# VITA-Group/CV_A-FAN

Measured on AMD Instinct MI355X. Metric: images/sec (whole node) A-FAN K=5 train step, ResNet-18/CIFAR-10, higher is better.
Workload: dtype bf16; 1 GPU; resnet18 CIFAR-10-shape A-FAN K=5 bf16, batch 256/GPU, perturb_idx 6, internal layout nhwc, 1xMI355X per rank (BASELINE configs[1]); global_batch=256, parallelism=dp1, hipgraph=True, in_launch_batchnorm=True

## Files before the change

### cv_a-fan_amd/csrc/afan_wgrad.hip

```cpp
#include "afan_common.h"
#include "afan_conv_stem.h"
#include "afan_wgrad_small.h"
#include <stdlib.h>

using namespace afan;

namespace {

typedef __bf16 bf16x8 __attribute__((ext_vector_type(8)));
typedef short s16x4 __attribute__((ext_vector_type(4)));
typedef float f32x16 __attribute__((ext_vector_type(16)));
typedef uint32_t u32x4 __attribute__((ext_vector_type(4)));

constexpr int THREADS = 256;
constexpr int BKP = 64;

struct FastDiv {
    uint32_t m, l;
};
static FastDiv make_fastdiv(uint32_t d) {
    FastDiv f;
    uint32_t l = 0;
    while ((1u << l) < d) ++l;
    f.l = l;
    f.m = (uint32_t)((((uint64_t)1 << 32) * (((uint64_t)1 << l) - d)) / d + 1);
    return f;
}
__device__ __forceinline__ uint32_t fdiv(uint32_t x, FastDiv f) { return (__umulhi(x, f.m) + x) >> f.l; }

struct WgradP {
    const uint16_t* x;
    const uint16_t* dy;
    float* slab;
    int N, Hi, Wi, Ci, Ho, Wo, Co;
    int k, stride, pad, dil;
    int S;
    int steps_per_slice;
    uint32_t P;
    FastDiv dWo, dHo;
    const uint16_t* x2;
    const uint16_t* dy2;
    uint32_t P1;
    int N2;
    int dn, dho, N1;
    int xcd_remap;
    float* direct;
    int accumulate;
};

template <int BM, int BN, bool INC>
__device__ __forceinline__ void wgrad_body(const WgradP& p, const uint32_t lin, const uint32_t tiles_, const uint32_t taps_,
                                           const uint32_t total) {
    constexpr int TM = BM / 2, TN = BN / 2, MI = TM / 32, NI = TN / 32;
    constexpr int LDA = BM + 32, LDB = BN + 32;
    constexpr int PA = BM / 8, PB = BN / 8;
    constexpr int RA = THREADS / PA, RB = THREADS / PB;
    constexpr int NA = BKP / RA, NB = BKP / RB;
    __shared__ __attribute__((aligned(16))) uint16_t As[BKP * LDA];
    __shared__ __attribute__((aligned(16))) uint16_t Bs[BKP * LDB];

    const int tid = threadIdx.x, lane = tid & 63, wave = tid >> 6;
    const int wr = wave >> 1, wc = wave & 1;
    const int tiles_n = (p.Ci + BN - 1) / BN;
    int tap, slice, tile;
    {
        uint32_t logical = lin;
        if (p.xcd_remap) {
            const uint32_t per = total >> 3, main_ = per << 3;
            if (lin < main_) logical = (lin & 7u) * per + (lin >> 3);
        }
        tap = (int)(logical % taps_);
        const uint32_t rest = logical / taps_;
        tile = (int)(rest % tiles_);
        slice = (int)(rest / tiles_);
    }
    const int co0 = (tile / tiles_n) * BM, ci0 = (tile % tiles_n) * BN;
    const int dh = (tap / p.k) * p.dil - p.pad, dw = (tap % p.k) * p.dil - p.pad;

    const __amdgpu_buffer_rsrc_t xr = __builtin_amdgcn_make_buffer_rsrc(
        const_cast<uint16_t*>(p.x), 0, (int)((int64_t)p.N * p.Hi * p.Wi * p.Ci * 2), 0x00020000);
    const __amdgpu_buffer_rsrc_t dr = __builtin_amdgcn_make_buffer_rsrc(
        const_cast<uint16_t*>(p.dy), 0, (int)((int64_t)p.P1 * p.Co * 2), 0x00020000);
    const __amdgpu_buffer_rsrc_t xr2 = __builtin_amdgcn_make_buffer_rsrc(
        const_cast<uint16_t*>(p.x2), 0, p.x2 ? (int)((int64_t)p.N2 * p.Hi * p.Wi * p.Ci * 2) : 0, 0x00020000);
    const __amdgpu_buffer_rsrc_t dr2 = __builtin_amdgcn_make_buffer_rsrc(
        const_cast<uint16_t*>(p.dy2), 0, p.dy2 ? (int)((int64_t)(p.P - p.P1) * p.Co * 2) : 0, 0x00020000);
    constexpr uint32_t OOB = 0x80000000u;

    const int pa = tid % PA, ra0 = tid / PA;
    const int pb = tid % PB, rb0 = tid / PB;
    const bool a_ok = co0 + pa * 8 < p.Co, b_ok = ci0 + pb * 8 < p.Ci;
    const uint32_t p_begin = (uint32_t)slice * p.steps_per_slice * BKP;

    f32x16 acc[MI][NI];
#pragma unroll
    for (int i = 0; i < MI; ++i)
#pragma unroll
        for (int j = 0; j < NI; ++j)
#pragma unroll
            for (int r = 0; r < 16; ++r) acc[i][j][r] = 0.f;

    u32x4 va[NA], vb[NB];
    int rn[NB], rho[NB];
    bool wi_ok[NB];
    uint32_t col_off[NB];
    if constexpr (INC) {
#pragma unroll
        for (int i = 0; i < NB; ++i) {
            const uint32_t pix = p_begin + rb0 + i * RB;
            const uint32_t t1 = fdiv(pix, p.dWo), wo = pix - t1 * p.Wo;
            const uint32_t n = fdiv(t1, p.dHo);
            rn[i] = (int)n;
            rho[i] = (int)(t1 - n * p.Ho);
            const int wi = (int)wo * p.stride + dw;
            wi_ok[i] = wi >= 0 && wi < p.Wi;
            col_off[i] = (uint32_t)((wi * p.Ci + ci0 + pb * 8) * 2);
        }
    }
    auto gload = [&](int ks) {
        const uint32_t pbase = p_begin + ks * BKP;
        const bool seg2 = pbase >= p.P1;
        const uint32_t shift = seg2 ? p.P1 : 0u, plim = seg2 ? p.P : p.P1;
        const __amdgpu_buffer_rsrc_t dsel = seg2 ? dr2 : dr, xsel = seg2 ? xr2 : xr;
#pragma unroll
        for (int i = 0; i < NA; ++i) {
            const uint32_t pix = pbase + ra0 + i * RA;
            const uint32_t off = (pix < plim && a_ok) ? ((pix - shift) * p.Co + co0 + pa * 8) * 2u : OOB;
            va[i] = __builtin_bit_cast(u32x4, __builtin_amdgcn_raw_buffer_load_b128(dsel, (int)off, 0, 0));
        }
#pragma unroll
        for (int i = 0; i < NB; ++i) {
            const uint32_t pix = pbase + rb0 + i * RB;
            if constexpr (INC) {
                const int hi = rho[i] * p.stride + dh;
                const int nl = rn[i] - (seg2 ? p.N1 : 0);
                const bool ok = pix < plim && wi_ok[i] && hi >= 0 && hi < p.Hi && b_ok;
                const uint32_t off = ok ? ((uint32_t)((nl * p.Hi + hi) * p.Wi) * (uint32_t)p.Ci) * 2u + col_off[i] : OOB;
                vb[i] = __builtin_bit_cast(u32x4, __builtin_amdgcn_raw_buffer_load_b128(xsel, (int)off, 0, 0));
                rn[i] += p.dn;
                rho[i] += p.dho;
                if (rho[i] >= p.Ho) { rho[i] -= p.Ho; rn[i] += 1; }
            } else {
                const uint32_t pl = pix - shift;
                const uint32_t t1 = fdiv(pl, p.dWo), wo = pl - t1 * p.Wo;
                const uint32_t n = fdiv(t1, p.dHo), ho = t1 - n * p.Ho;
                const int hi = (int)ho * p.stride + dh, wi = (int)wo * p.stride + dw;
                const bool ok = pix < plim && hi >= 0 && hi < p.Hi && wi >= 0 && wi < p.Wi && b_ok;
                const uint32_t off = ok ? (((n * p.Hi + hi) * p.Wi + wi) * p.Ci + ci0 + pb * 8) * 2u : OOB;
                vb[i] = __builtin_bit_cast(u32x4, __builtin_amdgcn_raw_buffer_load_b128(xsel, (int)off, 0, 0));
            }
        }
    };
    auto lstore = [&]() {
#pragma unroll
        for (int i = 0; i < NA; ++i) *reinterpret_cast<u32x4*>(As + (ra0 + i * RA) * LDA + pa * 8) = va[i];
#pragma unroll
        for (int i = 0; i < NB; ++i) *reinterpret_cast<u32x4*>(Bs + (rb0 + i * RB) * LDB + pb * 8) = vb[i];
    };
    const int fr = 8 * (lane >> 5) + ((lane & 15) >> 2);
    const int fc = 16 * ((lane >> 4) & 1) + 4 * (lane & 3);
    auto frag = [&](const uint16_t* T, int ld, int kbase, int cbase) -> bf16x8 {
        typedef s16x4 __attribute__((address_space(3))) * lptr;
        const uint16_t* a0 = T + (kbase + fr) * ld + cbase + fc;
        const s16x4 lo = __builtin_amdgcn_ds_read_tr16_b64_v4i16((lptr)(a0));
        const s16x4 hi = __builtin_amdgcn_ds_read_tr16_b64_v4i16((lptr)(a0 + 4 * ld));
        typedef short s16x8 __attribute__((ext_vector_type(8)));
        s16x8 v = {lo[0], lo[1], lo[2], lo[3], hi[0], hi[1], hi[2], hi[3]};
        return __builtin_bit_cast(bf16x8, v);
    };

    int KS = p.steps_per_slice;
    {
        const int64_t remaining = (int64_t)p.P - (int64_t)p_begin;
        const int64_t need = remaining <= 0 ? 0 : (remaining + BKP - 1) / BKP;
        if (need < KS) KS = (int)need;
    }
    if (KS > 0) gload(0);
    for (int ks = 0; ks < KS; ++ks) {
        lstore();
        __syncthreads();
        if (ks + 1 < KS) gload(ks + 1);
#pragma unroll
        for (int kk = 0; kk < BKP / 16; ++kk) {
            bf16x8 fa[MI], fb[NI];
#pragma unroll
            for (int i = 0; i < MI; ++i) fa[i] = frag(As, LDA, kk * 16, wr * TM + i * 32);
#pragma unroll
            for (int j = 0; j < NI; ++j) fb[j] = frag(Bs, LDB, kk * 16, wc * TN + j * 32);
#pragma unroll
            for (int i = 0; i < MI; ++i)
#pragma unroll
                for (int j = 0; j < NI; ++j)
                    acc[i][j] = __builtin_amdgcn_mfma_f32_32x32x16_bf16(fa[i], fb[j], acc[i][j], 0, 0, 0);
        }
        __syncthreads();
    }
    const int taps = p.k * p.k;
    float* out = p.slab + (((int64_t)slice * taps + tap) * p.Co) * p.Ci;
#pragma unroll
    for (int i = 0; i < MI; ++i)
#pragma unroll
        for (int j = 0; j < NI; ++j)
#pragma unroll
            for (int r = 0; r < 16; ++r) {
                const int co = co0 + wr * TM + i * 32 + (r & 3) + 8 * (r >> 2) + 4 * (lane >> 5);
                const int ci = ci0 + wc * TN + j * 32 + (lane & 31);
                if (co < p.Co && ci < p.Ci) {
                    if (p.direct) {
                        float* g = p.direct + ((int64_t)co * taps + tap) * p.Ci + ci;
                        *g = p.accumulate ? *g + acc[i][j][r] : acc[i][j][r];
                    } else {
                        out[(int64_t)co * p.Ci + ci] = acc[i][j][r];
                    }
                }
            }
}

template <int BM, int BN, bool INC>
__global__ __launch_bounds__(THREADS) void wgrad_kernel(const WgradP p) {
    wgrad_body<BM, BN, INC>(p, blockIdx.x + gridDim.x * (blockIdx.y + gridDim.y * blockIdx.z), gridDim.x, gridDim.y,
                            gridDim.x * gridDim.y * gridDim.z);
}

__device__ __forceinline__ f32x4 sum_slices(const float* __restrict__ p, int64_t stride, int S) {
    f32x4 s = {0.f, 0.f, 0.f, 0.f};
    int k = 0;
    for (; k + 8 <= S; k += 8) {
        f32x4 v[8];
#pragma unroll
        for (int u = 0; u < 8; ++u) v[u] = *reinterpret_cast<const f32x4*>(p + (int64_t)(k + u) * stride);
#pragma unroll
        for (int u = 0; u < 8; ++u) s += v[u];
    }
    for (; k < S; ++k) s += *reinterpret_cast<const f32x4*>(p + (int64_t)k * stride);
    return s;
}

constexpr int MAXQ = 4;
struct WgradPN {
    int n;
    uint32_t first[MAXQ + 1];
    uint32_t count[MAXQ];
    uint32_t tiles[MAXQ], taps[MAXQ];
    WgradP p[MAXQ];
};
template <int BM, int BN, bool INC>
__global__ __launch_bounds__(THREADS) void wgrad_multi_kernel(const WgradPN pn) {
    int q = 0;
    while (q + 1 < pn.n && blockIdx.x >= pn.first[q + 1]) ++q;
    const uint32_t lin = blockIdx.x - pn.first[q];
    if (lin >= pn.count[q]) return;
    wgrad_body<BM, BN, INC>(pn.p[q], lin, pn.tiles[q], pn.taps[q], pn.count[q]);
}

struct RedPN {
    const float* slab[MAXQ];
    float* grad[MAXQ];
    int S[MAXQ], taps[MAXQ], Co[MAXQ], Ci[MAXQ];
};
__global__ __launch_bounds__(THREADS) void wgrad_reduce_multi_kernel(const RedPN r, int accumulate) {
    const int q = blockIdx.y;
    const float* __restrict__ slab = r.slab[q];
    float* __restrict__ grad = r.grad[q];
    const int S = r.S[q], taps = r.taps[q], Co = r.Co[q], Ci = r.Ci[q];
    const int64_t per = (int64_t)taps * Co * Ci;
    const int64_t nvec = per / 4;
    for (int64_t v = (int64_t)blockIdx.x * THREADS + threadIdx.x; v < nvec; v += (int64_t)gridDim.x * THREADS) {
        const int64_t e = v * 4;
        const int ci = (int)(e % Ci);
        const int64_t t2 = e / Ci;
        const int co = (int)(t2 % Co);
        const int tap = (int)(t2 / Co);
        f32x4 s = sum_slices(slab + e, per, S);
        float* g = grad + ((int64_t)co * taps + tap) * Ci + ci;
        if (accumulate) s += *reinterpret_cast<const f32x4*>(g);
        *reinterpret_cast<f32x4*>(g) = s;
    }
}

__global__ __launch_bounds__(THREADS) void wgrad_reduce_kernel(const float* __restrict__ slab, float* __restrict__ grad,
                                                               int S, int taps, int Co, int Ci, int accumulate) {
    const int64_t per = (int64_t)taps * Co * Ci;
    const int64_t nvec = per / 4;
    for (int64_t v = (int64_t)blockIdx.x * THREADS + threadIdx.x; v < nvec; v += (int64_t)gridDim.x * THREADS) {
        const int64_t e = v * 4;
        const int ci = (int)(e % Ci);
        const int64_t t2 = e / Ci;
        const int co = (int)(t2 % Co);
        const int tap = (int)(t2 / Co);
        f32x4 s = sum_slices(slab + e, per, S);
        float* g = grad + ((int64_t)co * taps + tap) * Ci + ci;
        if (accumulate) s += *reinterpret_cast<const f32x4*>(g);
        *reinterpret_cast<f32x4*>(g) = s;
    }
}

struct Plan {
    int bm, bn, S, steps;
};

Plan make_plan(int64_t P, int co, int ci, int taps) {
    Plan pl;
    pl.bm = (co % 128 == 0) ? 128 : 64;
    pl.bn = (ci % 128 == 0) ? 128 : 64;
    const int64_t tiles = (int64_t)((co + pl.bm - 1) / pl.bm) * ((ci + pl.bn - 1) / pl.bn) * taps;
    const int64_t total_steps = (P + BKP - 1) / BKP;
    static const int target = [] { const char* v = getenv("AFAN_WGRAD_WGS"); return v ? atoi(v) : 512; }();
    int64_t S = target / tiles;
    static const int min_steps_env = [] { const char* v = getenv("AFAN_WGRAD_MINSTEPS"); return v ? atoi(v) : 0; }();
    const int min_steps = min_steps_env > 0 ? min_steps_env : (total_steps <= 40 ? 5 : 16);
    const int64_t max_s = total_steps / min_steps > 0 ? total_steps / min_steps : 1;
    if (S > max_s) S = max_s;
    if (S < 1) S = 1;
    static const int direct_on = [] { const char* v = getenv("AFAN_WGRAD_DIRECT"); return v ? atoi(v) : 0; }();
    if (direct_on && S == 2 && total_steps <= 64) S = 1;
    pl.steps = (int)((total_steps + S - 1) / S);
    pl.S = (int)((total_steps + pl.steps - 1) / pl.steps);
    return pl;
}

int build_problem(const void* x, const void* dy, int64_t n, const void* x2, const void* dy2, int64_t n2, float* grad, int64_t hi,
                  int64_t wi, int64_t ci, int64_t co, int k, int stride, int dilation, float* workspace, int accumulate,
                  WgradP& p, Plan& pl);

template <int BM, int BN>
int launch(const WgradP& p, int taps, hipStream_t st) {
    dim3 grid((unsigned)(((p.Co + BM - 1) / BM) * ((p.Ci + BN - 1) / BN)), (unsigned)taps, (unsigned)p.S);
    if (p.dn >= 0) wgrad_kernel<BM, BN, true><<<grid, THREADS, 0, st>>>(p);
    else wgrad_kernel<BM, BN, false><<<grid, THREADS, 0, st>>>(p);
    AFAN_LAUNCH_CHECK();
    AFAN_TRACE_LAUNCH("wgrad<%d,%d,inc%d>", BM, BN, p.dn >= 0 ? 1 : 0);
    return AFAN_OK;
}

}

extern "C" {

int64_t afan_conv_wgrad_workspace_floats(int64_t n, int64_t hi, int64_t wi, int64_t ci, int64_t co, int k, int stride) {
    if (ci == 3) return afan_stem::eligible(n, hi, wi, ci, co, k, stride) ? afan_stem::wgrad_workspace_floats(n, hi, wi, co) : 0;
    if (afan_wgrad_small::eligible(n, hi, wi, ci, co, k, stride)) return afan_wgrad_small::workspace_floats(n, hi, wi, ci, co, stride);
    if (n <= 0 || hi <= 0 || wi <= 0 || ci % 8 || co % 8 || ci < 40 || co < 40 || !(k == 1 || k == 3) || !(stride == 1 || stride == 2))
        return 0;
    const int pad = k / 2;
    const int64_t P = n * ((hi + 2 * pad - k) / stride + 1) * ((wi + 2 * pad - k) / stride + 1);
    const Plan pl = make_plan(P, (int)co, (int)ci, k * k);
    return (int64_t)pl.S * k * k * co * ci;
}

int afan_conv_wgrad_nhwc_bf16(const void* x, const void* dy, float* grad, int64_t n, int64_t hi, int64_t wi, int64_t ci,
                              int64_t co, int k, int stride, int dilation, float* workspace, int accumulate,
                              afan_stream_t stream) {
    return afan_conv_wgrad2_nhwc_bf16(x, dy, n, nullptr, nullptr, 0, grad, hi, wi, ci, co, k, stride, dilation, workspace,
                                      accumulate, stream);
}

int afan_conv_wgrad2_nhwc_bf16(const void* x, const void* dy, int64_t n, const void* x2, const void* dy2, int64_t n2,
                               float* grad, int64_t hi, int64_t wi, int64_t ci, int64_t co, int k, int stride, int dilation,
                               float* workspace, int accumulate, afan_stream_t stream) {
    if (n <= 0 || hi <= 0 || wi <= 0 || ci <= 0 || co <= 0 || n2 < 0) return AFAN_ESHAPE;
    AFAN_TRACE_PROBLEM(0, afan::trace::WGRAD, n + n2, hi, wi, ci, co, k, stride, dilation);
    if (dilation < 1 || (dilation > 1 && (k != 3 || stride != 1 || ci % 8 || co % 8 || ci < 40 || co < 40))) return AFAN_ESHAPE;
    if (n2 > 0 && ci == 3) return AFAN_ESHAPE;
    if (n2 > 0 && (!x2 || !dy2)) return AFAN_ENULL;
    if (ci == 3) {
        if (!afan_stem::eligible(n, hi, wi, ci, co, k, stride)) return AFAN_ESHAPE;
        if (!x || !dy || !grad || !workspace) return AFAN_ENULL;
        if (!aligned(dy, 16) || !aligned(grad, 4) || !aligned(workspace, 16)) return AFAN_EALIGN;
        hipStream_t st = (hipStream_t)stream;
        const double M = (double)n * hi * wi;
        AFAN_PROF_FLOPS("conv_stem_wgrad_kernel", 2.0 * (M * co + M * 3), 2.0 * M * co * 27, st);
        return afan_stem::wgrad_launch(x, dy, grad, n, hi, wi, co, workspace, accumulate, st);
    }
    if (dilation == 1 && afan_wgrad_small::eligible(n, hi, wi, ci, co, k, stride)) {
        if (!x || !dy || !grad || !workspace) return AFAN_ENULL;
        if (!aligned(x, 16) || !aligned(dy, 16) || !aligned(grad, 4) || !aligned(workspace, 16)) return AFAN_EALIGN;
        hipStream_t st = (hipStream_t)stream;
        const double P = (double)n * ((hi - 1) / stride + 1) * ((wi - 1) / stride + 1);
        AFAN_PROF_FLOPS("conv_wgrad_small_kernel", 2.0 * (P * co + (double)n * hi * wi * ci), 2.0 * P * co * ci * 9, st);
        if (n2 > 0 && (!aligned(x2, 16) || !aligned(dy2, 16))) return AFAN_EALIGN;
        return afan_wgrad_small::launch(x, dy, grad, n, hi, wi, ci, co, stride, workspace, accumulate, st, x2, dy2, n2);
    }
    WgradP p{};
    Plan pl;
    int e = build_problem(x, dy, n, x2, dy2, n2, grad, hi, wi, ci, co, k, stride, dilation, workspace, accumulate, p, pl);
    if (e) return e;
    const int taps = k * k;
    const int64_t P = (n + n2) * (int64_t)p.Ho * p.Wo;
    hipStream_t st = (hipStream_t)stream;
    int rc;
    {
        AFAN_PROF_FLOPS("conv_wgrad_kernel", 2.0 * (double)(P * co + n * hi * wi * ci) + 4.0 * pl.S * taps * co * ci,
                        2.0 * (double)P * co * ci * taps, st);
        if (pl.bm == 128) rc = pl.bn == 128 ? launch<128, 128>(p, taps, st) : launch<128, 64>(p, taps, st);
        else rc = pl.bn == 128 ? launch<64, 128>(p, taps, st) : launch<64, 64>(p, taps, st);
    }
    if (rc || p.direct) return rc;
    const int64_t per = (int64_t)taps * co * ci;
    AFAN_PROF("conv_wgrad_reduce_kernel", 4.0 * per * (pl.S + 1 + (accumulate ? 1 : 0)), st);
    wgrad_reduce_kernel<<<grid_for(per / 4, THREADS, 1024), THREADS, 0, st>>>(workspace, grad, pl.S, taps, (int)co, (int)ci,
                                                                              accumulate);
    AFAN_LAUNCH_CHECK();
    return AFAN_OK;
}

}

namespace {
int build_problem(const void* x, const void* dy, int64_t n, const void* x2, const void* dy2, int64_t n2, float* grad, int64_t hi,
                  int64_t wi, int64_t ci, int64_t co, int k, int stride, int dilation, float* workspace, int accumulate,
                  WgradP& p, Plan& pl) {
    if (ci % 8 || co % 8 || ci < 40 || co < 40 || !(k == 1 || k == 3) || !(stride == 1 || stride == 2)) return AFAN_ESHAPE;
    if (!x || !dy || !grad || !workspace) return AFAN_ENULL;
    if (!aligned(x, 16) || !aligned(dy, 16) || !aligned(grad, 16) || !aligned(workspace, 16)) return AFAN_EALIGN;
    const int pad = dilation * (k / 2);
    const int64_t ho = (hi + 2 * (k / 2) - k) / stride + 1, wo = (wi + 2 * (k / 2) - k) / stride + 1;
    const int64_t P1 = n * ho * wo, P = (n + n2) * ho * wo;
    if (P * co * 2 > 0x7fffffffLL || (n + n2) * hi * wi * ci * 2 > 0x7fffffffLL) return AFAN_ESHAPE;
    if (n2 > 0 && (P1 % BKP != 0 || !aligned(x2, 16) || !aligned(dy2, 16))) return n2 > 0 && P1 % BKP != 0 ? AFAN_ESHAPE : AFAN_EALIGN;
    const int taps = k * k;
    pl = make_plan(P, (int)co, (int)ci, taps);
    p.x = (const uint16_t*)x; p.dy = (const uint16_t*)dy; p.slab = workspace;
    p.N = (int)n; p.Hi = (int)hi; p.Wi = (int)wi; p.Ci = (int)ci; p.Ho = (int)ho; p.Wo = (int)wo; p.Co = (int)co;
    p.k = k; p.stride = stride; p.pad = pad; p.dil = dilation; p.S = pl.S; p.steps_per_slice = pl.steps; p.P = (uint32_t)P;
    p.x2 = (const uint16_t*)x2; p.dy2 = (const uint16_t*)dy2; p.P1 = (uint32_t)P1; p.N2 = (int)n2;
    p.N1 = (int)n;
    {
        static const bool remap_on = [] { const char* v = getenv("AFAN_WGRAD_XCD"); return !v || atoi(v) != 0; }();
        p.xcd_remap = remap_on ? 1 : 0;
    }
    p.dn = -1; p.dho = 0;
    {
        static const bool inc_on = [] { const char* v = getenv("AFAN_WGRAD_INC"); return !v || atoi(v) != 0; }();
        if (inc_on && BKP % wo == 0) {
            const int64_t hw = ho * wo;
            p.dn = (int)(BKP / hw);
            p.dho = (int)((BKP % hw) / wo);
        }
    }
    p.dWo = make_fastdiv((uint32_t)wo); p.dHo = make_fastdiv((uint32_t)ho);
    {
        static const int direct_on = [] { const char* v = getenv("AFAN_WGRAD_DIRECT"); return v ? atoi(v) : 0; }();
        p.direct = (direct_on && pl.S == 1) ? grad : nullptr;
        p.accumulate = accumulate;
    }
    return AFAN_OK;
}
}

extern "C" {

int afan_conv_wgrad_plan(int64_t n, int64_t hi, int64_t wi, int64_t ci, int64_t co, int k, int stride) {
    if (ci == 3 || afan_wgrad_small::eligible(n, hi, wi, ci, co, k, stride)) return 0;
    if (n <= 0 || hi <= 0 || wi <= 0 || ci % 8 || co % 8 || ci < 40 || co < 40 || !(k == 1 || k == 3) || !(stride == 1 || stride == 2))
        return 0;
    const int64_t ho = (hi + 2 * (k / 2) - k) / stride + 1, wo = (wi + 2 * (k / 2) - k) / stride + 1;
    const Plan pl = make_plan(n * ho * wo, (int)co, (int)ci, k * k);
    static const bool inc_on = [] { const char* v = getenv("AFAN_WGRAD_INC"); return !v || atoi(v) != 0; }();
    const int inc = (inc_on && BKP % wo == 0) ? 1 : 0;
    return pl.bm | (pl.bn << 8) | (inc << 16) | (1 << 17);
}

int afan_conv_wgrad_multi_nhwc_bf16(int nb, const void* const* x, const void* const* dy, float* const* grad, const int64_t* n,
                                    const int64_t* hi, const int64_t* wi, const int64_t* ci, const int64_t* co, const int* k,
                                    const int* stride, const int* dilation, float* workspace, int accumulate,
                                    afan_stream_t stream) {
    if (nb < 1 || nb > MAXQ) return AFAN_ESHAPE;
    if (!x || !dy || !grad || !n || !hi || !wi || !ci || !co || !k || !stride || !dilation || !workspace) return AFAN_ENULL;
    WgradPN pn{};
    RedPN rp{};
    pn.n = nb;
    int code0 = 0;
    int64_t woff = 0, max_vec = 0;
    double bytes = 0, flops = 0;
    for (int b = 0; b < nb; ++b) {
        const int code = afan_conv_wgrad_plan(n[b], hi[b], wi[b], ci[b], co[b], k[b], stride[b]);
        if (!code || (b && code != code0)) return AFAN_ESHAPE;
        code0 = code;
        if (dilation[b] < 1 || (dilation[b] > 1 && (k[b] != 3 || stride[b] != 1))) return AFAN_ESHAPE;
        AFAN_TRACE_PROBLEM(b, afan::trace::WGRAD, n[b], hi[b], wi[b], ci[b], co[b], k[b], stride[b], dilation[b]);
        Plan pl;
        int e = build_problem(x[b], dy[b], n[b], nullptr, nullptr, 0, grad[b], hi[b], wi[b], ci[b], co[b], k[b], stride[b],
                              dilation[b], workspace + woff, accumulate, pn.p[b], pl);
        if (e) return e;
        pn.p[b].direct = nullptr;
        const int taps = k[b] * k[b];
        const int bm = code & 0xff, bn = (code >> 8) & 0xff;
        pn.tiles[b] = (uint32_t)(((co[b] + bm - 1) / bm) * ((ci[b] + bn - 1) / bn));
        pn.taps[b] = (uint32_t)taps;
        pn.count[b] = pn.tiles[b] * taps * (uint32_t)pl.S;
        pn.first[b + 1] = (pn.first[b] + pn.count[b] + 7u) & ~7u;
        rp.slab[b] = workspace + woff; rp.grad[b] = grad[b]; rp.S[b] = pl.S; rp.taps[b] = taps; rp.Co[b] = (int)co[b]; rp.Ci[b] = (int)ci[b];
        const int64_t per = (int64_t)taps * co[b] * ci[b];
        woff += (int64_t)pl.S * per;
        if (per / 4 > max_vec) max_vec = per / 4;
        const double P = (double)n[b] * pn.p[b].Ho * pn.p[b].Wo;
        bytes += 2.0 * (P * co[b] + (double)n[b] * hi[b] * wi[b] * ci[b]) + 4.0 * pl.S * per;
        flops += 2.0 * P * co[b] * ci[b] * taps;
    }
    hipStream_t st = (hipStream_t)stream;
    const int bm = code0 & 0xff, bn = (code0 >> 8) & 0xff;
    const bool inc = (code0 >> 16) & 1;
    const unsigned G = pn.first[nb];
    {
    AFAN_PROF_FLOPS("conv_wgrad_kernel", bytes, flops, st);
#define AFAN_WM(BM_, BN_)                                                                                   \
    do {                                                                                                    \
        if (inc) wgrad_multi_kernel<BM_, BN_, true><<<G, THREADS, 0, st>>>(pn);                             \
        else wgrad_multi_kernel<BM_, BN_, false><<<G, THREADS, 0, st>>>(pn);                                \
    } while (0)
    if (bm == 128) { if (bn == 128) AFAN_WM(128, 128); else AFAN_WM(128, 64); }
    else { if (bn == 128) AFAN_WM(64, 128); else AFAN_WM(64, 64); }
#undef AFAN_WM
    AFAN_LAUNCH_CHECK();
    AFAN_TRACE_LAUNCH("wgrad_multi<%d,%d,inc%d>", bm, bn, inc ? 1 : 0);
    }
    AFAN_PROF("conv_wgrad_reduce_kernel", 4.0 * (double)woff, st);
    wgrad_reduce_multi_kernel<<<dim3((unsigned)grid_for(max_vec, THREADS, 1024), (unsigned)nb), THREADS, 0, st>>>(rp, accumulate);
    AFAN_LAUNCH_CHECK();
    return AFAN_OK;
}

}
```

Measured before the change: 33960 images/sec.

## Double-buffer LDS and register fragments in wgrad kernel; size split-K from occupancy

The wgrad MFMA kernel now keeps two LDS stages, so the next tile is stored and the one after is prefetched from global memory partway through the current tile's MFMA loop. This removes one of the two barriers per K step. LDS fragments are also double-buffered in registers, so reads for the next kk overlap the current MFMAs. The split-K workgroup target, previously a fixed 512, is now CUs times min(occupancy, 2), queried per tile shape. Doubled LDS and extra fragment registers may lower occupancy, and the getenv lookups are no longer cached statics, so they run on every plan call.

Result: slower. 33610 images/sec (-1.0%).

```diff
diff --git a/cv_a-fan_amd/csrc/afan_wgrad.hip b/cv_a-fan_amd/csrc/afan_wgrad.hip
--- a/cv_a-fan_amd/csrc/afan_wgrad.hip
+++ b/cv_a-fan_amd/csrc/afan_wgrad.hip
@@ -56,8 +56,8 @@
     constexpr int PA = BM / 8, PB = BN / 8;
     constexpr int RA = THREADS / PA, RB = THREADS / PB;
     constexpr int NA = BKP / RA, NB = BKP / RB;
-    __shared__ __attribute__((aligned(16))) uint16_t As[BKP * LDA];
-    __shared__ __attribute__((aligned(16))) uint16_t Bs[BKP * LDB];
+    __shared__ __attribute__((aligned(16))) uint16_t As[2 * BKP * LDA];
+    __shared__ __attribute__((aligned(16))) uint16_t Bs[2 * BKP * LDB];
 
     const int tid = threadIdx.x, lane = tid & 63, wave = tid >> 6;
     const int wr = wave >> 1, wc = wave & 1;
@@ -151,11 +151,13 @@
             }
         }
     };
-    auto lstore = [&]() {
-#pragma unroll
-        for (int i = 0; i < NA; ++i) *reinterpret_cast<u32x4*>(As + (ra0 + i * RA) * LDA + pa * 8) = va[i];
-#pragma unroll
-        for (int i = 0; i < NB; ++i) *reinterpret_cast<u32x4*>(Bs + (rb0 + i * RB) * LDB + pb * 8) = vb[i];
+    auto lstore = [&](int stage) {
+        uint16_t* A = As + stage * (BKP * LDA);
+        uint16_t* B = Bs + stage * (BKP * LDB);
+#pragma unroll
+        for (int i = 0; i < NA; ++i) *reinterpret_cast<u32x4*>(A + (ra0 + i * RA) * LDA + pa * 8) = va[i];
+#pragma unroll
+        for (int i = 0; i < NB; ++i) *reinterpret_cast<u32x4*>(B + (rb0 + i * RB) * LDB + pb * 8) = vb[i];
     };
     const int fr = 8 * (lane >> 5) + ((lane & 15) >> 2);
     const int fc = 16 * ((lane >> 4) & 1) + 4 * (lane & 3);
@@ -175,23 +177,38 @@
         const int64_t need = remaining <= 0 ? 0 : (remaining + BKP - 1) / BKP;
         if (need < KS) KS = (int)need;
     }
-    if (KS > 0) gload(0);
+    if (KS > 0) {
+        gload(0);
+        lstore(0);
+        if (KS > 1) gload(1);
+    }
+    __syncthreads();
     for (int ks = 0; ks < KS; ++ks) {
-        lstore();
-        __syncthreads();
-        if (ks + 1 < KS) gload(ks + 1);
+        const int cur = ks & 1;
+        const uint16_t* A = As + cur * (BKP * LDA);
+        const uint16_t* B = Bs + cur * (BKP * LDB);
+        bf16x8 fa[2][MI], fb[2][NI];
+#pragma unroll
+        for (int i = 0; i < MI; ++i) fa[0][i] = frag(A, LDA, 0, wr * TM + i * 32);
+#pragma unroll
+        for (int j = 0; j < NI; ++j) fb[0][j] = frag(B, LDB, 0, wc * TN + j * 32);
 #pragma unroll
         for (int kk = 0; kk < BKP / 16; ++kk) {
-            bf16x8 fa[MI], fb[NI];
-#pragma unroll
-            for (int i = 0; i < MI; ++i) fa[i] = frag(As, LDA, kk * 16, wr * TM + i * 32);
-#pragma unroll
-            for (int j = 0; j < NI; ++j) fb[j] = frag(Bs, LDB, kk * 16, wc * TN + j * 32);
+            if (kk + 1 < BKP / 16) {
+#pragma unroll
+                for (int i = 0; i < MI; ++i) fa[(kk + 1) & 1][i] = frag(A, LDA, (kk + 1) * 16, wr * TM + i * 32);
+#pragma unroll
+                for (int j = 0; j < NI; ++j) fb[(kk + 1) & 1][j] = frag(B, LDB, (kk + 1) * 16, wc * TN + j * 32);
+            }
 #pragma unroll
             for (int i = 0; i < MI; ++i)
 #pragma unroll
                 for (int j = 0; j < NI; ++j)
-                    acc[i][j] = __builtin_amdgcn_mfma_f32_32x32x16_bf16(fa[i], fb[j], acc[i][j], 0, 0, 0);
+                    acc[i][j] = __builtin_amdgcn_mfma_f32_32x32x16_bf16(fa[kk & 1][i], fb[kk & 1][j], acc[i][j], 0, 0, 0);
+            if (kk == BKP / 32 - 1 && ks + 1 < KS) {
+                lstore(cur ^ 1);
+                if (ks + 2 < KS) gload(ks + 2);
+            }
         }
         __syncthreads();
     }
@@ -299,15 +316,42 @@
     int bm, bn, S, steps;
 };
 
+template <int BM, int BN>
+int chip_holds() {
+    static const int v = [] {
+        int dev = 0, cus = 0, occ = 1 << 30;
+        const void* ks[4] = {(const void*)wgrad_kernel<BM, BN, true>, (const void*)wgrad_kernel<BM, BN, false>,
+                             (const void*)wgrad_multi_kernel<BM, BN, true>, (const void*)wgrad_multi_kernel<BM, BN, false>};
+        if (hipGetDevice(&dev) != hipSuccess || hipDeviceGetAttribute(&cus, hipDeviceAttributeMultiprocessorCount, dev) != hipSuccess ||
+            cus <= 0) {
+            (void)hipGetLastError();
+            return 512;
+        }
+        for (const void* k : ks) {
+            int o = 0;
+            if (hipOccupancyMaxActiveBlocksPerMultiprocessor(&o, k, THREADS, 0) != hipSuccess || o < 1) {
+                (void)hipGetLastError();
+                return 512;
+            }
+            if (o < occ) occ = o;
+        }
+        return cus * (occ < 2 ? occ : 2);
+    }();
+    return v;
+}
+
 Plan make_plan(int64_t P, int co, int ci, int taps) {
     Plan pl;
     pl.bm = (co % 128 == 0) ? 128 : 64;
     pl.bn = (ci % 128 == 0) ? 128 : 64;
     const int64_t tiles = (int64_t)((co + pl.bm - 1) / pl.bm) * ((ci + pl.bn - 1) / pl.bn) * taps;
     const int64_t total_steps = (P + BKP - 1) / BKP;
-    static const int target = [] { const char* v = getenv("AFAN_WGRAD_WGS"); return v ? atoi(v) : 512; }();
+    const int target_env = [] { const char* v = getenv("AFAN_WGRAD_WGS"); return v ? atoi(v) : 0; }();
+    const int target = target_env > 0 ? target_env
+                                      : (pl.bm == 128 ? (pl.bn == 128 ? chip_holds<128, 128>() : chip_holds<128, 64>())
+                                                      : (pl.bn == 128 ? chip_holds<64, 128>() : chip_holds<64, 64>()));
     int64_t S = target / tiles;
-    static const int min_steps_env = [] { const char* v = getenv("AFAN_WGRAD_MINSTEPS"); return v ? atoi(v) : 0; }();
+    const int min_steps_env = [] { const char* v = getenv("AFAN_WGRAD_MINSTEPS"); return v ? atoi(v) : 0; }();
     const int min_steps = min_steps_env > 0 ? min_steps_env : (total_steps <= 40 ? 5 : 16);
     const int64_t max_s = total_steps / min_steps > 0 ? total_steps / min_steps : 1;
     if (S > max_s) S = max_s;
```
